# EleutherAI/DALLE-mtf

Hardware: AMD Instinct MI355X
Metric: train tokens/sec (text+image) per node, dalle_example (higher is better)
Workload: dtype bf16

## Files before the change

dalle-mtf_amd/csrc/attention.hip:

```cpp
#include "common.h"
#include <type_traits>
#include <algorithm>
#include <string.h>
#include <vector>

#define HD 128
#define LOG2E_F 1.4426950408889634f
#define KP 136
#define TP 68
#define TP32 36

__device__ __forceinline__ bf16x8 cat4(bf16x4 a, bf16x4 b) { return __builtin_shufflevector(a, b, 0, 1, 2, 3, 4, 5, 6, 7); }
__device__ __forceinline__ bf16x8 pack_bf8(const float* p) {
  u32x4 v = {pack2bf(p[0], p[1]), pack2bf(p[2], p[3]), pack2bf(p[4], p[5]), pack2bf(p[6], p[7])};
  return __builtin_bit_cast(bf16x8, v);
}

template <int ROWS>
__device__ __forceinline__ void load_nat_regs(u32x4* r, const bf16_t* __restrict__ g, int64_t ld, int row0, int nrows, int tid) {
#pragma unroll
  for (int i = 0; i < ROWS / 16; ++i) {
    const int c = tid + 256 * i, row = c >> 4, ch = c & 15;
    int gr = row0 + row;
    gr = gr < nrows ? gr : nrows - 1;
// ... 836 lines not shown
  {
    const int items = ((S + 127) / 128) * B * H;
    const int grid = items < 2 * attn_num_cus() ? items : 2 * attn_num_cus();
    const int perxcd = g_opt_attn_xcd && (B * H) % 8 == 0 && grid % 8 == 0;
    if (g_opt_attn_fwd == 0) attn_fwd_kernel<false><<<dim3(grid), dim3(256), 2 * QK_STAGE, (hipStream_t)stream>>>(qkv, o, lse, B, H, S, perxcd);
#ifdef ATTN_STAMP
    else attn_fwd2_kernel<<<dim3(grid), dim3(256), 2 * QK_STAGE, (hipStream_t)stream>>>(qkv, o, lse, B, H, S, perxcd, g_dbg_buf);
#else
    else attn_fwd2_kernel<<<dim3(grid), dim3(256), 2 * QK_STAGE, (hipStream_t)stream>>>(qkv, o, lse, B, H, S, perxcd);
#endif
  }
  DMI_CHECK_LAUNCH("attention_fwd");
  return DMI_OK;
}

template <int rowstore, bool MASKED, typename... PLAN>
__global__ __launch_bounds__(256, 2) void attn_bwd_dq_kernel(const bf16_t* __restrict__ qkv, const bf16_t* __restrict__ o,
                                                             const bf16_t* __restrict__ d_o, const float* __restrict__ lse,
                                                             float* __restrict__ delta, float* __restrict__ stats,
                                                             bf16_t* __restrict__ dqkv, PLAN __restrict__... plan_, int B, int H, int S, int perxcd) {
  static_assert(sizeof...(PLAN) == (MASKED ? 1 : 0), "the plan pointer is an argument of the masked instance only");
  extern __shared__ __attribute__((aligned(16))) char sm[];
  const int d = H * HD, ld3 = 3 * d;
  int T = (S + 127) / 128, W = 0;
  const int* __restrict__ fptr = nullptr;
  const int* __restrict__ flist = nullptr;
  const int* __restrict__ forder = nullptr;
  const unsigned* __restrict__ rowbits = nullptr;
  if constexpr (MASKED) {
    const int* __restrict__ plan = (plan_, ...);
    T = plan[AMP_NB], W = plan[AMP_W];
    fptr = plan + plan[AMP_FPTR];
    flist = plan + plan[AMP_FLIST];
    forder = plan + plan[AMP_FORDER];
    rowbits = (const unsigned*)(plan + plan[AMP_ROWBITS]);
  }
  const AttnSched sched = attn_sched(T, B * H, perxcd);
  int tile_, bh;
  for (int round = 0; attn_item(sched, round, tile_, bh); ++round) {
// ... 11 lines not shown
  int tid = threadIdx.x;
  asm volatile("" : "+v"(tid));
  const int lane = tid & 63;
  const int wid = __builtin_amdgcn_readfirstlane(tid >> 6);
  const int r = lane & 31, h = lane >> 5, g4 = lane >> 4, l16 = lane & 15;
  const int qrow = q0 + wid * 32 + r;
  const int qrow_c = qrow < S ? qrow : S - 1;
  const unsigned* __restrict__ mrow = nullptr;
  if constexpr (MASKED) mrow = rowbits + (int64_t)qrow_c * W;
  const bf16_t* qb = qkv + (int64_t)b * S * ld3 + hh * HD;
  const bf16_t* dob = d_o + (int64_t)b * S * d + hh * HD;
  const unsigned lds0 = (unsigned)(uintptr_t)(__attribute__((address_space(3))) char*)sm;
  const int nbytes = (int)(((int64_t)(S - 1) * ld3 + HD) * 2);
  const __amdgpu_buffer_rsrc_t rk = __builtin_amdgcn_make_buffer_rsrc((void*)(qb + d), 0, nbytes, 0x00020000);
  const __amdgpu_buffer_rsrc_t rv = __builtin_amdgcn_make_buffer_rsrc((void*)(qb + 2 * d), 0, nbytes, 0x00020000);

  bf16x8 qf[8], dof[8], of_[8];
#pragma unroll
  for (int kk = 0; kk < 8; ++kk) {
    qf[kk] = *(const bf16x8*)(qb + (int64_t)qrow_c * ld3 + 16 * kk + 8 * h);
    dof[kk] = *(const bf16x8*)(dob + (int64_t)qrow_c * d + 16 * kk + 8 * h);
    of_[kk] = *(const bf16x8*)(o + ((int64_t)b * S + qrow_c) * d + hh * HD + 16 * kk + 8 * h);
  }
  const float lse_q = lse[(int64_t)bh * S + qrow_c];
  const float lse2_q = lse_q * LOG2E_F;
  float delta_q = 0.f;
  {
#pragma unroll
    for (int kk = 0; kk < 8; ++kk) {
      float fo[8], fd[8];
      unpack8(__builtin_bit_cast(u32x4, of_[kk]), fo);
      unpack8(__builtin_bit_cast(u32x4, dof[kk]), fd);
#pragma unroll
      for (int j = 0; j < 8; ++j) delta_q += fo[j] * fd[j];
    }
    delta_q += __shfl_xor(delta_q, 32, 64);
    if (h == 0 && qrow < S) {
      const int64_t idx = (int64_t)bh * S + qrow;
      delta[idx] = delta_q;
      stats[2 * idx] = lse2_q;
      stats[2 * idx + 1] = delta_q;
    }
  }

  int vo[4];
#pragma unroll
  for (int i = 0; i < 4; ++i) {
    const int c = tid + 256 * i, row = c >> 4, pc = c & 15;
    vo[i] = (row * ld3 + 8 * (pc ^ swz(row))) * 2;
  }
  auto stage = [&](int st, int key0) {
    char* base = sm + st * QK_STAGE;
#pragma unroll
    for (int i = 0; i < 4; ++i) {
      dma16(rk, base + (wid * 64 + 256 * i) * 16, vo[i] + key0 * ld3 * 2);
      dma16(rv, base + 16384 + (wid * 64 + 256 * i) * 16, vo[i] + key0 * ld3 * 2);
    }
  };
  int ofa[8];
#pragma unroll
  for (int kk = 0; kk < 8; ++kk) ofa[kk] = r * 256 + (((2 * kk + h) ^ swz(r)) << 4);
  const int rr = l16 >> 2;
  unsigned oft0[2];
#pragma unroll
  for (int w2 = 0; w2 < 2; ++w2) {
    const int row = 4 * h + rr + 8 * w2;
    const int chunk = 2 * (g4 & 1) + ((l16 & 3) >> 1);
    oft0[w2] = row * 256 + ((chunk ^ swz(row)) << 4) + 8 * (l16 & 1);
  }

  f32x16 dq[4];
#pragma unroll
// ... 51 lines not shown
      } else {
#pragma unroll
        for (int e = 0; e < 16; ++e) {
          const float pe = __builtin_amdgcn_exp2f(__builtin_fmaf(s[e], LOG2E_F, -lse2_q));
          ds[e] = pe * (dp[e] - delta_q);
        }
      }
      bf16x8 dsb[2];
      dsb[0] = pack_bf8(ds);
      dsb[1] = pack_bf8(ds + 8);
#pragma unroll
      for (int q = 0; q < 4; ++q) {
        const int s2 = q >> 1, dp2 = (q & 1) * 2;
        Tr2& c = tk[q & 1];
        tr2_wait(c);
        if (q < 3) {
          const int s2n = (q + 1) >> 1, dn = ((q + 1) & 1) * 2;
          const unsigned u0 = t0 + s2n * 4096, u1 = t1 + s2n * 4096;
          tr2_issue(tk[(q + 1) & 1], lds0 + (u0 ^ (dn << 6)), lds0 + (u1 ^ (dn << 6)), lds0 + (u0 ^ ((dn + 1) << 6)), lds0 + (u1 ^ ((dn + 1) << 6)));
        }
        dq[dp2] = __builtin_amdgcn_mfma_f32_32x32x16_bf16(cat2(c.a0, c.a1), dsb[s2], dq[dp2], 0, 0, 0);
        dq[dp2 + 1] = __builtin_amdgcn_mfma_f32_32x32x16_bf16(cat2(c.b0, c.b1), dsb[s2], dq[dp2 + 1], 0, 0, 0);
      }
    }
  };

  if constexpr (MASKED) {
    if (nsteps > 0) stage(0, 64 * (list[0] & 0xffff));
    asm volatile("s_waitcnt vmcnt(0)" ::: "memory");
    __syncthreads();
    for (int i = 0; i < nsteps; ++i) {
      const int ent = list[i];
      unsigned b0, b1;
      amp_row_bits(ent, wid, mrow, W, b0, b1);
      if (i + 1 < nsteps) stage((i + 1) & 1, 64 * (list[i + 1] & 0xffff));
      compute(i & 1, ent, b0, b1);
      asm volatile("s_waitcnt vmcnt(0)" ::: "memory");
      __syncthreads();
    }
  } else {
    stage(0, 0);
    asm volatile("s_waitcnt vmcnt(0)" ::: "memory");
    __syncthreads();
    int j = 0;
    for (; j + 2 <= nsteps; j += 2) {
      stage(1, 64 * (j + 1));
      compute(0, j);
      asm volatile("s_waitcnt vmcnt(0)" ::: "memory");
      __syncthreads();
      if (j + 2 < nsteps) stage(0, 64 * (j + 2));
      compute(1, j + 1);
      asm volatile("s_waitcnt vmcnt(0)" ::: "memory");
      __syncthreads();
// ... 38 lines not shown
      "ds_read_b128 %4, %8 offset:128\n\t"
      "ds_read_b128 %5, %8 offset:144\n\t"
      "ds_read_b128 %6, %8 offset:192\n\t"
      "ds_read_b128 %7, %8 offset:208"
      : "=&v"(f.v[0]), "=&v"(f.v[1]), "=&v"(f.v[2]), "=&v"(f.v[3]), "=&v"(f.v[4]), "=&v"(f.v[5]), "=&v"(f.v[6]), "=&v"(f.v[7])
      : "v"(a)
      : "memory");
}
template <int N>
__device__ __forceinline__ void st8_wait(St8& f) {
  asm volatile("s_waitcnt lgkmcnt(%8)"
               : "+v"(f.v[0]), "+v"(f.v[1]), "+v"(f.v[2]), "+v"(f.v[3]), "+v"(f.v[4]), "+v"(f.v[5]), "+v"(f.v[6]), "+v"(f.v[7])
               : "n"(N)
               : "memory");
}
template <int rowstore>
__global__ __launch_bounds__(256, 1) void attn_bwd_dkv_kernel(const bf16_t* __restrict__ qkv, const bf16_t* __restrict__ d_o,
                                                               const float* __restrict__ stats ,
                                                               bf16_t* __restrict__ dqkv, int B, int H, int S, int perxcd) {
  extern __shared__ __attribute__((aligned(16))) char sm[];
  const int d = H * HD, ld3 = 3 * d;
  const AttnSched sched = attn_sched((S + 127) / 128, B * H, perxcd);
  int ktile, bh;
  for (int round = 0; attn_item(sched, round, ktile, bh); ++round) {
  const int b = bh / H, hh = bh % H;
  const int key0 = ktile * 128;
  int tid = threadIdx.x;
  asm volatile("" : "+v"(tid));
  const int lane = tid & 63;
  const int wid = __builtin_amdgcn_readfirstlane(tid >> 6);
  const int r = lane & 31, h = lane >> 5, g4 = lane >> 4, l16 = lane & 15;
  const int krow = key0 + wid * 32 + r;
  const int krow_c = krow < S ? krow : S - 1;
  const bf16_t* qb = qkv + (int64_t)b * S * ld3 + hh * HD;
  const bf16_t* kb = qb + d;
  const bf16_t* vb = qb + 2 * d;
  const bf16_t* dob = d_o + (int64_t)b * S * d + hh * HD;
  const unsigned lds0 = (unsigned)(uintptr_t)(__attribute__((address_space(3))) char*)sm;

  const __amdgpu_buffer_rsrc_t rq = __builtin_amdgcn_make_buffer_rsrc((void*)qb, 0, (int)(((int64_t)(S - 1) * ld3 + HD) * 2), 0x00020000);
  const __amdgpu_buffer_rsrc_t rdo = __builtin_amdgcn_make_buffer_rsrc((void*)dob, 0, (int)(((int64_t)(S - 1) * d + HD) * 2), 0x00020000);
  const __amdgpu_buffer_rsrc_t rv = __builtin_amdgcn_make_buffer_rsrc((void*)vb, 0, (int)(((int64_t)(S - 1) * ld3 + HD) * 2), 0x00020000);
  const __amdgpu_buffer_rsrc_t rst = __builtin_amdgcn_make_buffer_rsrc((void*)(stats + (int64_t)bh * S * 2), 0, S * 8, 0x00020000);

  bf16x8 kf[8];
#pragma unroll
  for (int kk = 0; kk < 8; ++kk) kf[kk] = *(const bf16x8*)(kb + (int64_t)krow_c * ld3 + 16 * kk + 8 * h);

#pragma unroll
  for (int i = 0; i < 8; ++i) {
    const int c = tid + 256 * i, row = c >> 4, pc = c & 15;
    int gr = key0 + row;
    gr = gr < S ? gr : S - 1;
    dma16(rv, sm + (wid * 64 + 256 * i) * 16, (gr * ld3 + 8 * (pc ^ swz(row))) * 2);
  }
  int voq[2], vod[2];
#pragma unroll
  for (int i = 0; i < 2; ++i) {
// ... 146 lines not shown
      if (do_dma) stage_q(st3, q3, 1);
      dk[2] = __builtin_amdgcn_mfma_f32_32x32x16_bf16(cat2(tq.c0, tq.c1), dsb[0], dk[2], 0, 0, 0);
      dk[3] = __builtin_amdgcn_mfma_f32_32x32x16_bf16(cat2(tq.d0, tq.d1), dsb[0], dk[3], 0, 0, 0);
      __builtin_amdgcn_sched_barrier(0);
      tr4_wait8(t2, tq);
      if constexpr (has_next) st8_issue(stt, lds0 + 32768 + so + 16384 + 32 * h);
      dv[0] = __builtin_amdgcn_mfma_f32_32x32x16_bf16(cat2(t2.a0, t2.a1), pb[1], dv[0], 0, 0, 0);
      dv[1] = __builtin_amdgcn_mfma_f32_32x32x16_bf16(cat2(t2.b0, t2.b1), pb[1], dv[1], 0, 0, 0);
      if (do_dma) stage_st(st3, q3);
      dv[2] = __builtin_amdgcn_mfma_f32_32x32x16_bf16(cat2(t2.c0, t2.c1), pb[1], dv[2], 0, 0, 0);
      dv[3] = __builtin_amdgcn_mfma_f32_32x32x16_bf16(cat2(t2.d0, t2.d1), pb[1], dv[3], 0, 0, 0);
      __builtin_amdgcn_sched_barrier(0);
      if constexpr (has_next) tr4_wait8(tdo, t2); else tr4_wait(tdo);
      dk[0] = __builtin_amdgcn_mfma_f32_32x32x16_bf16(cat2(tdo.a0, tdo.a1), dsb[1], dk[0], 0, 0, 0);
      dk[1] = __builtin_amdgcn_mfma_f32_32x32x16_bf16(cat2(tdo.b0, tdo.b1), dsb[1], dk[1], 0, 0, 0);
      dk[2] = __builtin_amdgcn_mfma_f32_32x32x16_bf16(cat2(tdo.c0, tdo.c1), dsb[1], dk[2], 0, 0, 0);
      dk[3] = __builtin_amdgcn_mfma_f32_32x32x16_bf16(cat2(tdo.d0, tdo.d1), dsb[1], dk[3], 0, 0, 0);
      if constexpr (has_next) st8_wait<0>(stt);
    }
  };

  if (nsteps > 0) stage(0, 32 * qi0);
  if (nsteps > 1) stage(1, 32 * (qi0 + 1));
  if (nsteps > 2) stage(2, 32 * (qi0 + 2));
  if (nsteps > 2) DKV_WAIT(5); else DKV_WAIT(0);
  DKV_BARRIER();
  if (nsteps > 0) {
    st8_issue(stt, lds0 + 32768 + 16384 + 32 * h);
    sdp_only(0, sA, dpA);
  }
  int t = 0;
#define DKV_STEP(CS, CD, NS, ND, NEXT, MASK)                                \
  {                                                                         \
    body(t & 3, qi0 + t, t, CS, CD, NS, ND, std::integral_constant<bool, NEXT>{}, std::integral_constant<bool, MASK>{}); \
    if (nsteps - 1 - t >= 3) DKV_WAIT(5); else DKV_WAIT(0);                 \
    DKV_BARRIER();                                                          \
    ++t;                                                                    \
  }
  while (t < 4 && t + 3 <= nsteps) {
    DKV_STEP(sA, dpA, sB, dpB, true, true) DKV_STEP(sB, dpB, sA, dpA, true, true)
  }
  while (t + 3 <= nsteps) {
    DKV_STEP(sA, dpA, sB, dpB, true, false) DKV_STEP(sB, dpB, sA, dpA, true, false)
  }
  if (nsteps - t == 2) {
    DKV_STEP(sA, dpA, sB, dpB, true, true) DKV_STEP(sB, dpB, sA, dpA, false, true)
  } else if (nsteps - t == 1) {
    DKV_STEP(sA, dpA, sB, dpB, false, true)
  }
#undef DKV_STEP
// ... 6 lines not shown
    __syncthreads();
  } else if (krow < S) {
    bf16_t* okp = dqkv + ((int64_t)b * S + krow) * ld3 + d + hh * HD;
    bf16_t* ovp = okp + d;
#pragma unroll
    for (int dt = 0; dt < 4; ++dt)
#pragma unroll
      for (int q4 = 0; q4 < 4; ++q4) {
        const int dd = dt * 32 + 8 * q4 + 4 * h;
        *(u32x2*)(okp + dd) = u32x2{pack2bf(dk[dt][4 * q4], dk[dt][4 * q4 + 1]), pack2bf(dk[dt][4 * q4 + 2], dk[dt][4 * q4 + 3])};
        *(u32x2*)(ovp + dd) = u32x2{pack2bf(dv[dt][4 * q4], dv[dt][4 * q4 + 1]), pack2bf(dv[dt][4 * q4 + 2], dv[dt][4 * q4 + 3])};
      }
  }
  }
}

extern "C" int dmi_attention_bwd(const uint16_t* qkv, const uint16_t* o, const uint16_t* d_o, const float* lse, float* delta,
                                 uint16_t* dqkv, int B, int H, int S, void* stream) {
  DMI_REQUIRE(qkv && o && d_o && lse && delta && dqkv, "attention_bwd: null pointer");
  DMI_REQUIRE(B > 0 && H > 0 && S > 0 && S % 8 == 0, "attention_bwd: S must be a multiple of 8 (S=%d)", S);
  DMI_REQUIRE((int64_t)S * 3 * H * HD * 2 < 0x7fffffff, "attention_bwd: sequence too long for 32-bit buffer offsets");
  hipStream_t st = (hipStream_t)stream;
  float* stats = delta + (int64_t)B * H * S;
  static bool attr_done = false;
  const int shm = 32768 + DKV_NSTAGE * DKV_STAGE;
  if (!attr_done) {
    (void)hipFuncSetAttribute((const void*)attn_bwd_dq_kernel<0, false>, hipFuncAttributeMaxDynamicSharedMemorySize, 2 * QK_STAGE);
    (void)hipFuncSetAttribute((const void*)attn_bwd_dq_kernel<1, false>, hipFuncAttributeMaxDynamicSharedMemorySize, 2 * QK_STAGE);
    (void)hipFuncSetAttribute((const void*)attn_bwd_dkv_kernel<0>, hipFuncAttributeMaxDynamicSharedMemorySize, shm);
    (void)hipFuncSetAttribute((const void*)attn_bwd_dkv_kernel<1>, hipFuncAttributeMaxDynamicSharedMemorySize, shm);
    attr_done = true;
  }
  const int items = ((S + 127) / 128) * B * H;
  {
    const int grid = items < 2 * attn_num_cus() ? items : 2 * attn_num_cus();
    const int perxcd = g_opt_attn_xcd && (B * H) % 8 == 0 && grid % 8 == 0;
    if (g_opt_attn_bwd & 1) attn_bwd_dq_kernel<1, false><<<dim3(grid), dim3(256), 2 * QK_STAGE, st>>>(qkv, o, d_o, lse, delta, stats, dqkv, B, H, S, perxcd);
    else attn_bwd_dq_kernel<0, false><<<dim3(grid), dim3(256), 2 * QK_STAGE, st>>>(qkv, o, d_o, lse, delta, stats, dqkv, B, H, S, perxcd);
  }
  DMI_CHECK_LAUNCH("attention_bwd_dq");
  {
    const int grid = items < attn_num_cus() ? items : attn_num_cus();
    const int perxcd = g_opt_attn_xcd && (B * H) % 8 == 0 && grid % 8 == 0;
    if (g_opt_attn_bwd & 1) attn_bwd_dkv_kernel<1><<<dim3(grid), dim3(256), shm, st>>>(qkv, d_o, stats, dqkv, B, H, S, perxcd);
    else attn_bwd_dkv_kernel<0><<<dim3(grid), dim3(256), shm, st>>>(qkv, d_o, stats, dqkv, B, H, S, perxcd);
  }
  DMI_CHECK_LAUNCH("attention_bwd_dkv");
  return DMI_OK;
}

#define DEC_WAVES 16
template <int STRIDE>
__device__ __forceinline__ float lane_groups_sum(float v) {
  if constexpr (STRIDE < 64) {
    v += __shfl_xor(v, STRIDE, 64);
    return lane_groups_sum<2 * STRIDE>(v);
  }
  return v;
}
template <int HEAD_DIM, bool MASKED, typename... PLAN>
__global__ __launch_bounds__(64 * DEC_WAVES) void attn_decode_kernel(bf16_t* qkv, const bf16_t* __restrict__ fresh, bf16_t* __restrict__ o,
                                                                     PLAN __restrict__... plan_, int H, int S, int pos_arg,
                                                                     const int* __restrict__ pos_dev) {
// ... 1111 lines not shown
```

dalle-mtf_amd/csrc/gemm.hip:

```cpp
#include "common.h"
#include <string.h>
#include <type_traits>

static int g_opt_nt4 = 1;
static int g_opt_nt8 = 1;
int g_opt_reserve_cus = 0;
int g_opt_attn_fwd = 1;
int g_opt_attn_bwd = 1;
int g_opt_attn_mask_force = 0;
int g_opt_attn_xcd = 8;
static int g_opt_tn8 = 0;
static int g_opt_tn8_max_tiles = 16;
static int g_opt_nt8_min_k = 2048;
static int g_opt_skinny = 1;
static int g_opt_tn_wide = 1;
static int g_opt_tn_tail = 1;
static int g_opt_cstream = 1;
static int g_opt_cstream_min_mb = 256;
static int g_opt_cstream_nt_min_mb = 1024;
static int g_opt_res16 = 1;
static int g_opt_ntr = 1;
static int g_opt_nt8p = 1;
static int g_opt_relu_bits = 1;
static int g_opt_nt8p_max_k = 1024;
// ... 3315 lines not shown
```

dalle-mtf_amd/dalle_hip/__init__.py:

```python
from __future__ import annotations

import ctypes
import os
import re
import struct

import numpy as np
from ctypes import c_char_p, c_float, c_int, c_int64, c_uint64, c_void_p

import torch

_HERE = os.path.dirname(os.path.abspath(__file__))
LIB_PATH = os.environ.get("DALLE_HIP_LIB") or os.path.join(_HERE, "libdalle_hip.so")
HEADER_PATH = os.path.join(os.path.dirname(os.path.dirname(_HERE)), "include", "dalle_hip.h")

GEMM_BIAS, GEMM_RELU, GEMM_RESIDUAL, GEMM_RELU_MASK, GEMM_OUT_F32, GEMM_ROWSCALE = 1, 2, 4, 8, 16, 32
GEMM_GELU = 512

_lib = None


class DalleHipError(RuntimeError):
    pass

# ... 52 lines not shown
        "dmi_gemm_nt_splitk_workspace_bytes": (L64, [I, I, I]),
        "dmi_gemm_nt_splitk": (I, [P, I, P, I, P, I, I, I, I, P, P, P]),
        "dmi_gemm_tn_workspace_bytes": (L64, [I, I, I]),
        "dmi_gemm_tn": (I, [P, I, P, I, P, P, P, I, I, I, P, P, P, P]),
        "dmi_gemm_tn_group": (I, [P, I, I, P, P, P]),
        "dmi_gemm_tn_group_plan": (I, [P, P, I, I]),
        "dmi_reduce_slabs_batch": (I, [P, I, P]),
        "dmi_colsum_workspace_bytes": (L64, [L64, I]),
        "dmi_colsum": (I, [P, I, P, L64, I, P, P]),
        "dmi_transpose_bf16": (I, [P, P, I, I, I, P]),
        "dmi_attention_fwd": (I, [P, P, P, I, I, I, P]),
        "dmi_attention_bwd": (I, [P, P, P, P, P, P, I, I, I, P]),
        "dmi_attention_decode": (I, [P, P, P, I, I, I, I, P, P]),
        "dmi_attention_fwd_hd": (I, [P, P, P, I, I, I, I, P]),
        "dmi_attention_bwd_hd": (I, [P, P, P, P, P, P, I, I, I, I, P]),
        "dmi_attention_decode_hd": (I, [P, P, P, I, I, I, I, P, I, P]),
        "dmi_attn_mask_plan": (L64, [P, I, P, L64]),
        "dmi_attention_fwd_masked": (I, [P, P, P, P, P, I, I, I, I, P]),
        "dmi_attention_bwd_masked": (I, [P, P, P, P, P, P, P, P, I, I, I, I, P]),
        "dmi_attention_decode_masked": (I, [P, P, P, P, P, I, I, I, I, P, I, P]),
        "dmi_label_logit": (I, [P, I, P, I, P, P, P, P, L64, I, I, P]),
        "dmi_gemm_nt_softmax_partials": (L64, [I]),
        "dmi_gemm_nt_softmax": (I, [P, I, P, I, P, P, P, I, P, I, I, I, P]),
        "dmi_softmax_finish": (I, [P, I, P, P, P, P, I, P, I, P, P, I, I, P, P, P, P, P, L64, I, I, F, P]),
        "dmi_softmax_finish_w": (I, [P, I, P, P, P, P, I, P, I, P, P, I, I, P, P, P, P, P, L64, I, I, F, P, I, P]),
        "dmi_loss_reduce": (I, [P, L64, P, I, I, F, P, P]),
        "dmi_shift_labels": (I, [P, P, I, I, I, P]),
        "dmi_cross_entropy": (I, [P, I, P, P, P, L64, I, F, P]),
        "dmi_sum_f32": (I, [P, L64, F, P, P]),
        "dmi_assemble_tokens": (I, [P, P, P, I, I, I, I, I, P]),
# ... 428 lines not shown
    _dev(in_base, out_base, table)
    _check(lib().dmi_transpose_bf16_batch(_p(in_base), _p(out_base), _p(table), n, total_tiles, _stream()), "transpose_batch")


def attention_fwd(qkv, o, lse, B, H, S, head_dim=128):
    _dev(qkv, o, lse)
    _check(lib().dmi_attention_fwd_hd(_p(qkv), _p(o), _p(lse), B, H, S, int(head_dim), _stream()), "attention_fwd")


def attention_bwd(qkv, o, d_o, lse, scratch, dqkv, B, H, S, head_dim=128):
    _dev(qkv, o, d_o, lse, scratch, dqkv)
    _check(lib().dmi_attention_bwd_hd(_p(qkv), _p(o), _p(d_o), _p(lse), _p(scratch), _p(dqkv), B, H, S, int(head_dim), _stream()),
           "attention_bwd")


PLAN_MAGIC = 0x504D4144
PLAN_HDR = dict(S=1, NB=2, W=3, CAUSAL=4, FPTR=5, FLIST=6, KPTR=7, KLIST=8, FORDER=9, KORDER=10, ROWBITS=11, COLBITS=12, WORDS=13,
                LIVE_F=14, CAUSAL_F=15, LIVE_K=16, CAUSAL_K=17)


class AttnMaskPlan:

    def __init__(self, mask, device="cuda"):
        m = np.ascontiguousarray(np.asarray(mask.cpu() if hasattr(mask, "cpu") else mask).astype(np.uint8))
        if m.ndim != 2 or m.shape[0] != m.shape[1]:
            raise DalleHipError(f"attn_mask_plan: the mask must be [S, S] (got {m.shape})")
        self.S = int(m.shape[0])
        fn = lib().dmi_attn_mask_plan
        nbytes = fn(m.ctypes.data, self.S, None, 0)
        if nbytes < 0:
# ... 357 lines not shown
```

dalle-mtf_amd/src/dalle_mtf/engine.py:

```python
from __future__ import annotations

import contextlib
import gc
import hashlib
import logging
import math
import os
from collections import OrderedDict, namedtuple
from typing import Dict, Optional, Tuple

import numpy as np
import torch

import dalle_hip as dh
from ..dp import GradReducer
from .activations import check_activation
from .dropout import SITE_POSITION, SITE_TOKEN, resolve_dropout, site_attention, site_key, site_mlp
from .layout import ALIGN, ParamLayout, _round_up, adafactor_factored_dims, adafactor_table, reference_init
from .ff_glu import resolve_ff_glu
from .qk_norm import GAIN_NAMES, resolve_qk_norm
from .ema import ema_decay_at, one_minus_decay, resolve_ema, resolve_weights
from .loss_weights import position_weights, resolve_loss_weights
from .rotary import DEFAULT_BASE, resolve_rotary, rotary_table
from .token_shift import grid_side, resolve_token_shift
# ... 147 lines not shown
            if plan.causal:
                continue
            if self.hd != 128:
                raise dh.DalleHipError(f"custom attention masks need head dim 128 (n_embd/n_heads = {self.hd}); "
                                       "the head-dim-64 kernels implement the causal mask only")
            self.attn_plan[l] = plan

    def _attn_fwd(self, l, qkv, o, lse):
        if self.attn_plan[l] is None:
            dh.attention_fwd(qkv, o, lse, self.B, self.H, self.S, head_dim=self.hd)
        else:
            dh.attention_fwd_masked(qkv, o, lse, self.attn_plan[l], self.B, self.H, self.S, head_dim=self.hd)

    def _attn_bwd(self, l):
        args = (self.qkv[l], self.o[l], self.d_o, self.lse[l], self.delta, self.dqkv)
        if self.attn_plan[l] is None:
            dh.attention_bwd(*args, self.B, self.H, self.S, head_dim=self.hd)
        else:
            dh.attention_bwd_masked(*args, self.attn_plan[l], self.B, self.H, self.S, head_dim=self.hd)

    def _attn_decode(self, l, cache, o, fresh, pos_dev):
        if self.attn_plan[l] is None:
            dh.attention_decode(cache, o, self.B, self.H, self.S, 0, fresh=fresh, pos_dev=pos_dev, head_dim=self.hd)
        else:
            dh.attention_decode_masked(cache, o, self.attn_plan[l], self.B, self.H, self.S, 0, fresh=fresh, pos_dev=pos_dev,
                                       head_dim=self.hd)

    OPTIMIZERS = ("adam", "adafactor")

    def set_optimizer(self, name):
        name = (name or "adam").lower()
# ... 191 lines not shown
        self.tok_sorted = torch.empty(M, dtype=torch.int32, device=self.dev)
        self.tok_perm = torch.empty(M, dtype=torch.int32, device=self.dev)
        self.sort_ws = torch.empty(dh.sort_tokens_workspace_bytes(M), **u8)
        self.embed_ws = torch.empty(dh.embed_bwd_workspace_bytes(B, S, d), **u8)
        self.sort_stream = torch.cuda.Stream(device=self.dev)
        self._sort_done = None
        self.dx = [torch.empty(M, d, **b16) for _ in range(2)]
        self.dxn = torch.empty(M, d, **b16)
        self.dh = torch.empty(M, 4 * d, **b16)
        self.dpre = torch.empty(M, self.F1, **b16) if self.ffn_form == "glu" else None
        self.dqkv = torch.empty(M, 3 * d, **b16)
        self.d_o = torch.empty(M, d, **b16)
        self.drop_y = torch.empty(M, d, **b16) if self.resid_thresh else None
        self.dyd = [torch.empty(M, d, **b16) for _ in range(2)] if self.resid_thresh else None
        self.delta = torch.empty(3, B, H, S, **f32)
        wsz = max(dh.gemm_tn_workspace_bytes(M, d, Vp), *(dh.gemm_tn_workspace_bytes(M, i_, j_) for i_, j_ in self.wgrad_shapes),
                  dh.layernorm_bwd_workspace_bytes(M, d), dh.sumsq_workspace_bytes(self.lay.total),
                  dh.gemm_nt_splitk_workspace_bytes(M // 2 + 256, d, 8),
                  dh.qk_norm_bwd_workspace_bytes(M, self.hd) if self.qk_norm else 0)
        self.ws = torch.empty(int(wsz) + 1024, **u8)
        self.ws_blk = [torch.empty(int(dh.gemm_tn_workspace_bytes(M, i_, j_)) + 256, **u8) for i_, j_ in self.wgrad_shapes]
        self.deferred = dh.DeferredReduces()
        if self.fuse_lnbwd:
            npart = dh.gemm_nt_lnbwd_parts(M) * 2 * d
            self.lnb_part = [torch.empty(npart, **f32) for _ in range(2 * L if self.lnb_batch else 1)]
            self.ln_ws_final = torch.empty(int(dh.layernorm_bwd_workspace_bytes(M, d)) + 256, **u8)

    def _w(self, name):
        return self.view(self.pb, name)

# ... 712 lines not shown
```

include/dalle_hip.h:

```cpp
#ifndef DALLE_HIP_H
#define DALLE_HIP_H
#include <stddef.h>
#include <stdint.h>
#ifdef __cplusplus
extern "C" {
#endif

typedef enum {
  DMI_OK = 0,
  DMI_ERR_INVALID = -1,
  DMI_ERR_LAUNCH = -2,
  DMI_ERR_UNSUPPORTED = -3
} dmi_status;

const char* dmi_last_error_string(void);
int dmi_version(void);
int dmi_get_option(const char* name);
int dmi_set_option(const char* name, int value);
int dmi_set_debug_buffer(void* device_buffer);

int dmi_embed_fwd(const int32_t* tokens, const uint16_t* wte, const uint16_t* wpe, uint16_t* x,
                  int64_t rows , int S, int d, int vocab, const int* pos_dev, void* stream);
int64_t dmi_sort_tokens_workspace_bytes(int64_t n);
int dmi_sort_tokens(const int32_t* tokens, int32_t* sorted_tokens, int32_t* perm, int64_t n, int vocab,
// ... 57 lines not shown
                const uint16_t* bias_weights, int M, int I, int J, void* workspace, dmi_reduce_item* deferred,
                int* n_deferred, void* stream);
int dmi_reduce_slabs_batch(const dmi_reduce_item* items, int n, void* stream);
typedef struct dmi_tn_problem { const uint16_t* X; int ldx; const uint16_t* dY; int ldy; float* dW; float* dbias;
                                const uint16_t* bias_weights; int I; int J; void* workspace; } dmi_tn_problem;
int dmi_gemm_tn_group(const dmi_tn_problem* probs, int n, int M, dmi_reduce_item* deferred, int* n_deferred, void* stream);
int dmi_gemm_tn_group_plan(const int* I, const int* J, int n, int M);

int64_t dmi_colsum_workspace_bytes(int64_t M, int N);
int dmi_colsum(const uint16_t* Y, int ldy, float* out, int64_t M, int N, void* workspace, void* stream);
int dmi_transpose_bf16(const uint16_t* in, uint16_t* out, int batch, int R, int C, void* stream);

int dmi_attention_fwd(const uint16_t* qkv, uint16_t* o, float* lse, int B, int H, int S, void* stream);
int dmi_attention_bwd(const uint16_t* qkv, const uint16_t* o, const uint16_t* d_o, const float* lse, float* scratch,
                      uint16_t* dqkv, int B, int H, int S, void* stream);

int dmi_attention_decode(uint16_t* qkv, const uint16_t* fresh, uint16_t* o, int B, int H, int S, int pos, const int* pos_dev,
                         void* stream);
int dmi_attention_fwd_hd(const uint16_t* qkv, uint16_t* o, float* lse, int B, int H, int S, int head_dim, void* stream);
int dmi_attention_bwd_hd(const uint16_t* qkv, const uint16_t* o, const uint16_t* d_o, const float* lse, float* scratch,
                         uint16_t* dqkv, int B, int H, int S, int head_dim, void* stream);
int dmi_attention_decode_hd(uint16_t* qkv, const uint16_t* fresh, uint16_t* o, int B, int H, int S, int pos, const int* pos_dev,
                            int head_dim, void* stream);

int64_t dmi_attn_mask_plan(const uint8_t* mask, int S, int32_t* plan, int64_t plan_bytes);
int dmi_attention_fwd_masked(const uint16_t* qkv, uint16_t* o, float* lse, const int32_t* plan, const int32_t* plan_host, int B, int H,
                             int S, int head_dim, void* stream);
int dmi_attention_bwd_masked(const uint16_t* qkv, const uint16_t* o, const uint16_t* d_o, const float* lse, float* scratch,
                             uint16_t* dqkv, const int32_t* plan, const int32_t* plan_host, int B, int H, int S, int head_dim,
                             void* stream);
// ... 133 lines not shown
```

Measured before the change: 2.812 million.

## Reuse dS from dK/dV backward pass in dQ kernel via workspace

Restructures the causal attention backward. A separate delta kernel computes the row statistics first. The dK/dV kernel then writes its bf16 dS tiles into a per-(batch, head) global workspace, and a new dQ kernel variant streams K and those stored dS tiles instead of recomputing QK^T, softmax and dP. This removes the duplicated score and dP recomputation in the dQ pass. In exchange it adds global-memory writes and reads of the dS tiles, a large extra workspace allocation, and one more kernel launch. It is enabled by default through the option value change and the engine allocating the workspace.

Result: no change. 2.834 million, median of 6 (+0.8%).

```diff
diff --git a/dalle-mtf_amd/csrc/attention.hip b/dalle-mtf_amd/csrc/attention.hip
--- a/dalle-mtf_amd/csrc/attention.hip
+++ b/dalle-mtf_amd/csrc/attention.hip
@@ -874,15 +874,28 @@
   return DMI_OK;
 }
 
-template <int rowstore, bool MASKED, typename... PLAN>
+#define DS_SUB 2048
+#ifndef DS_STORE_AUX
+#define DS_STORE_AUX 18
+#endif
+#define DS_SLOTS 2
+__host__ __device__ __forceinline__ int ds_sub_base(int kb, int nq32) { return 4 * (kb * nq32 - 2 * kb * (kb - 1)); }
+__device__ __forceinline__ void dma16_s(__amdgpu_buffer_rsrc_t rsrc, char* lds_wave_base, int voff, int soff) {
+  __builtin_amdgcn_raw_ptr_buffer_load_lds(rsrc, (__attribute__((address_space(3))) void*)lds_wave_base, 16, voff, soff, 0, 0);
+}
+template <int form, bool MASKED, typename... PLAN>
 __global__ __launch_bounds__(256, 2) void attn_bwd_dq_kernel(const bf16_t* __restrict__ qkv, const bf16_t* __restrict__ o,
                                                              const bf16_t* __restrict__ d_o, const float* __restrict__ lse,
                                                              float* __restrict__ delta, float* __restrict__ stats,
                                                              bf16_t* __restrict__ dqkv, PLAN __restrict__... plan_, int B, int H, int S, int perxcd) {
-  static_assert(sizeof...(PLAN) == (MASKED ? 1 : 0), "the plan pointer is an argument of the masked instance only");
+  constexpr int rowstore = form & 1;
+  constexpr bool DS = (form & 2) != 0;
+  static_assert(!(DS && MASKED) && (!DS || rowstore), "dQ from dS: the causal whole-row-store instance only");
+  static_assert(sizeof...(PLAN) == (MASKED || DS ? 1 : 0), "the plan / workspace pointer is an argument of the masked / dS instance only");
   extern __shared__ __attribute__((aligned(16))) char sm[];
   const int d = H * HD, ld3 = 3 * d;
   int T = (S + 127) / 128, W = 0;
+  [[maybe_unused]] const int nq32 = (S + 31) / 32;
   const int* __restrict__ fptr = nullptr;
   const int* __restrict__ flist = nullptr;
   const int* __restrict__ forder = nullptr;
@@ -924,8 +937,15 @@
   const int nbytes = (int)(((int64_t)(S - 1) * ld3 + HD) * 2);
   const __amdgpu_buffer_rsrc_t rk = __builtin_amdgcn_make_buffer_rsrc((void*)(qb + d), 0, nbytes, 0x00020000);
   const __amdgpu_buffer_rsrc_t rv = __builtin_amdgcn_make_buffer_rsrc((void*)(qb + 2 * d), 0, nbytes, 0x00020000);
+  [[maybe_unused]] __amdgpu_buffer_rsrc_t rds = rv;
+  if constexpr (DS) {
+    const int ds_bytes = ds_sub_base(T, nq32) * DS_SUB;
+    rds = __builtin_amdgcn_make_buffer_rsrc((void*)((const char*)(plan_, ...) + (int64_t)bh * ds_bytes), 0, ds_bytes, 0x00020000);
+  }
 
   bf16x8 qf[8], dof[8], of_[8];
+  float lse2_q = 0.f, delta_q = 0.f;
+  if constexpr (!DS) {
 #pragma unroll
   for (int kk = 0; kk < 8; ++kk) {
     qf[kk] = *(const bf16x8*)(qb + (int64_t)qrow_c * ld3 + 16 * kk + 8 * h);
@@ -933,8 +953,7 @@
     of_[kk] = *(const bf16x8*)(o + ((int64_t)b * S + qrow_c) * d + hh * HD + 16 * kk + 8 * h);
   }
   const float lse_q = lse[(int64_t)bh * S + qrow_c];
-  const float lse2_q = lse_q * LOG2E_F;
-  float delta_q = 0.f;
+  lse2_q = lse_q * LOG2E_F;
   {
 #pragma unroll
     for (int kk = 0; kk < 8; ++kk) {
@@ -952,6 +971,7 @@
       stats[2 * idx + 1] = delta_q;
     }
   }
+  }
 
   int vo[4];
 #pragma unroll
@@ -966,6 +986,22 @@
       dma16(rk, base + (wid * 64 + 256 * i) * 16, vo[i] + key0 * ld3 * 2);
       dma16(rv, base + 16384 + (wid * 64 + 256 * i) * 16, vo[i] + key0 * ld3 * 2);
     }
+  };
+  [[maybe_unused]] const int qi = 4 * qt + wid;
+  auto ds_live = [&](int j) { return qi < nq32 && 2 * j <= qi; };
+  auto stage_k = [&](int st, int j) {
+#pragma unroll
+    for (int i = 0; i < 4; ++i) dma16(rk, sm + st * 16384 + (wid * 64 + 256 * i) * 16, vo[i] + 64 * j * ld3 * 2);
+  };
+  auto stage_ds = [&](int slot, int j) {
+    const int kb = j >> 1;
+#ifdef ATTN_DBG_DS_CONST
+    const int soff = 0 * kb;
+#else
+    const int soff = (ds_sub_base(kb, nq32) + (qi - 4 * kb) * 4 + 2 * (j & 1)) * DS_SUB;
+#endif
+#pragma unroll
+    for (int i = 0; i < 4; ++i) dma16_s(rds, sm + 32768 + slot * 16384 + wid * 4096 + i * 1024, lane * 16 + i * 1024, soff);
   };
   int ofa[8];
 #pragma unroll
@@ -1047,6 +1083,39 @@
         const int s2 = q >> 1, dp2 = (q & 1) * 2;
         Tr2& c = tk[q & 1];
         tr2_wait(c);
+        if (q < 3) {
+          const int s2n = (q + 1) >> 1, dn = ((q + 1) & 1) * 2;
+          const unsigned u0 = t0 + s2n * 4096, u1 = t1 + s2n * 4096;
+          tr2_issue(tk[(q + 1) & 1], lds0 + (u0 ^ (dn << 6)), lds0 + (u1 ^ (dn << 6)), lds0 + (u0 ^ ((dn + 1) << 6)), lds0 + (u1 ^ ((dn + 1) << 6)));
+        }
+        dq[dp2] = __builtin_amdgcn_mfma_f32_32x32x16_bf16(cat2(c.a0, c.a1), dsb[s2], dq[dp2], 0, 0, 0);
+        dq[dp2 + 1] = __builtin_amdgcn_mfma_f32_32x32x16_bf16(cat2(c.b0, c.b1), dsb[s2], dq[dp2 + 1], 0, 0, 0);
+      }
+    }
+  };
+
+  auto compute_ds = [&](int st, int slot, int j) {
+    if (!ds_live(j)) return;
+    const unsigned ods = lds0 + 32768 + slot * 16384 + wid * 4096 + (g4 & 1) * 1024 + (4 * h + rr) * 32 + (l16 & 1) * 16 + ((l16 & 3) >> 1) * 8;
+#pragma unroll
+    for (int kt2 = 0; kt2 < 2; ++kt2) {
+      Tr2 dsf, tk[2];
+      tr2_issue(dsf, ods + kt2 * DS_SUB, ods + kt2 * DS_SUB + 256, ods + kt2 * DS_SUB + 512, ods + kt2 * DS_SUB + 768);
+      unsigned ob = st * 16384 + kt2 * 8192;
+      asm volatile("" : "+v"(ob));
+      const unsigned t0 = ob + oft0[0], t1 = ob + oft0[1];
+      tr2_issue(tk[0], lds0 + t0, lds0 + t1, lds0 + (t0 ^ 64u), lds0 + (t1 ^ 64u));
+      bf16x8 dsb[2];
+#pragma unroll
+      for (int q = 0; q < 4; ++q) {
+        const int s2 = q >> 1, dp2 = (q & 1) * 2;
+        Tr2& c = tk[q & 1];
+        tr2_wait(c);
+        if (q == 0) {
+          tr2_wait(dsf);
+          dsb[0] = cat2(dsf.a0, dsf.a1);
+          dsb[1] = cat2(dsf.b0, dsf.b1);
+        }
         if (q < 3) {
           const int s2n = (q + 1) >> 1, dn = ((q + 1) & 1) * 2;
           const unsigned u0 = t0 + s2n * 4096, u1 = t1 + s2n * 4096;
@@ -1070,6 +1139,20 @@
       compute(i & 1, ent, b0, b1);
       asm volatile("s_waitcnt vmcnt(0)" ::: "memory");
       __syncthreads();
+    }
+  } else if constexpr (DS) {
+    stage_k(0, 0);
+    if (ds_live(0)) stage_ds(0, 0);
+    asm volatile("s_waitcnt vmcnt(0)" ::: "memory");
+    __syncthreads();
+    for (int j = 0; j < nsteps; ++j) {
+      if (j + 1 < nsteps) {
+        stage_k((j + 1) & 1, j + 1);
+        if (ds_live(j + 1)) stage_ds((j + 1) & 1, j + 1);
+      }
+      compute_ds(j & 1, j & 1, j);
+      asm volatile("s_waitcnt vmcnt(0)" ::: "memory");
+      if (j + 1 < nsteps) __syncthreads();
     }
   } else {
     stage(0, 0);
@@ -1138,10 +1221,10 @@
                : "n"(N)
                : "memory");
 }
-template <int rowstore>
-__global__ __launch_bounds__(256, 1) void attn_bwd_dkv_kernel(const bf16_t* __restrict__ qkv, const bf16_t* __restrict__ d_o,
-                                                               const float* __restrict__ stats ,
-                                                               bf16_t* __restrict__ dqkv, int B, int H, int S, int perxcd) {
+template <int rowstore, bool DS>
+__device__ __forceinline__ void attn_bwd_dkv_body(const bf16_t* __restrict__ qkv, const bf16_t* __restrict__ d_o,
+                                                  const float* __restrict__ stats ,
+                                                  bf16_t* __restrict__ dqkv, char* __restrict__ ws, int B, int H, int S, int perxcd) {
   extern __shared__ __attribute__((aligned(16))) char sm[];
   const int d = H * HD, ld3 = 3 * d;
   const AttnSched sched = attn_sched((S + 127) / 128, B * H, perxcd);
@@ -1166,6 +1249,14 @@
   const __amdgpu_buffer_rsrc_t rdo = __builtin_amdgcn_make_buffer_rsrc((void*)dob, 0, (int)(((int64_t)(S - 1) * d + HD) * 2), 0x00020000);
   const __amdgpu_buffer_rsrc_t rv = __builtin_amdgcn_make_buffer_rsrc((void*)vb, 0, (int)(((int64_t)(S - 1) * ld3 + HD) * 2), 0x00020000);
   const __amdgpu_buffer_rsrc_t rst = __builtin_amdgcn_make_buffer_rsrc((void*)(stats + (int64_t)bh * S * 2), 0, S * 8, 0x00020000);
+  [[maybe_unused]] __amdgpu_buffer_rsrc_t rws = rst;
+  [[maybe_unused]] int ws_item = 0;
+  if constexpr (DS) {
+    const int nq32 = (S + 31) / 32;
+    const int ds_bytes = ds_sub_base((S + 127) / 128, nq32) * DS_SUB;
+    rws = __builtin_amdgcn_make_buffer_rsrc((void*)(ws + (int64_t)bh * ds_bytes), 0, ds_bytes, 0x00020000);
+    ws_item = (ds_sub_base(ktile, nq32) + wid) * DS_SUB;
+  }
 
   bf16x8 kf[8];
 #pragma unroll
@@ -1342,6 +1433,11 @@
       if constexpr (has_next) tr4_wait8(tdo, t2); else tr4_wait(tdo);
       dk[0] = __builtin_amdgcn_mfma_f32_32x32x16_bf16(cat2(tdo.a0, tdo.a1), dsb[1], dk[0], 0, 0, 0);
       dk[1] = __builtin_amdgcn_mfma_f32_32x32x16_bf16(cat2(tdo.b0, tdo.b1), dsb[1], dk[1], 0, 0, 0);
+      if constexpr (DS) {
+        const int so_ds = ws_item + t * (4 * DS_SUB);
+        __builtin_amdgcn_raw_buffer_store_b128(__builtin_bit_cast(u32x4, dsb[0]), rws, r * 32 + h * 16, so_ds, DS_STORE_AUX);
+        __builtin_amdgcn_raw_buffer_store_b128(__builtin_bit_cast(u32x4, dsb[1]), rws, r * 32 + h * 16 + 1024, so_ds, DS_STORE_AUX);
+      }
       dk[2] = __builtin_amdgcn_mfma_f32_32x32x16_bf16(cat2(tdo.c0, tdo.c1), dsb[1], dk[2], 0, 0, 0);
       dk[3] = __builtin_amdgcn_mfma_f32_32x32x16_bf16(cat2(tdo.d0, tdo.d1), dsb[1], dk[3], 0, 0, 0);
       if constexpr (has_next) st8_wait<0>(stt);
@@ -1361,7 +1457,8 @@
 #define DKV_STEP(CS, CD, NS, ND, NEXT, MASK)                                \
   {                                                                         \
     body(t & 3, qi0 + t, t, CS, CD, NS, ND, std::integral_constant<bool, NEXT>{}, std::integral_constant<bool, MASK>{}); \
-    if (nsteps - 1 - t >= 3) DKV_WAIT(5); else DKV_WAIT(0);                 \
+    if constexpr (DS) { if (nsteps - 1 - t >= 3) DKV_WAIT(7); else DKV_WAIT(2); }  \
+    else { if (nsteps - 1 - t >= 3) DKV_WAIT(5); else DKV_WAIT(0); }          \
     DKV_BARRIER();                                                          \
     ++t;                                                                    \
   }
@@ -1398,12 +1495,69 @@
   }
   }
 }
-
-extern "C" int dmi_attention_bwd(const uint16_t* qkv, const uint16_t* o, const uint16_t* d_o, const float* lse, float* delta,
-                                 uint16_t* dqkv, int B, int H, int S, void* stream) {
-  DMI_REQUIRE(qkv && o && d_o && lse && delta && dqkv, "attention_bwd: null pointer");
-  DMI_REQUIRE(B > 0 && H > 0 && S > 0 && S % 8 == 0, "attention_bwd: S must be a multiple of 8 (S=%d)", S);
-  DMI_REQUIRE((int64_t)S * 3 * H * HD * 2 < 0x7fffffff, "attention_bwd: sequence too long for 32-bit buffer offsets");
+template <int rowstore>
+__global__ __launch_bounds__(256, 1) void attn_bwd_dkv_kernel(const bf16_t* __restrict__ qkv, const bf16_t* __restrict__ d_o,
+                                                               const float* __restrict__ stats, bf16_t* __restrict__ dqkv, int B, int H,
+                                                               int S, int perxcd) {
+  attn_bwd_dkv_body<rowstore, false>(qkv, d_o, stats, dqkv, nullptr, B, H, S, perxcd);
+}
+__global__ __launch_bounds__(256, 1) void attn_bwd_dkv_ds_kernel(const bf16_t* __restrict__ qkv, const bf16_t* __restrict__ d_o,
+                                                                  const float* __restrict__ stats, bf16_t* __restrict__ dqkv,
+                                                                  char* __restrict__ ws, int B, int H, int S, int perxcd) {
+  attn_bwd_dkv_body<1, true>(qkv, d_o, stats, dqkv, ws, B, H, S, perxcd);
+}
+
+__global__ __launch_bounds__(256) void attn_bwd_delta_kernel(const bf16_t* __restrict__ o, const bf16_t* __restrict__ d_o,
+                                                             const float* __restrict__ lse, float* __restrict__ delta,
+                                                             float* __restrict__ stats, int B, int H, int S) {
+  __shared__ u32x4 img[4][2][512];
+  const int lane = threadIdx.x & 63, wid = threadIdx.x >> 6;
+  const int64_t nseg = (int64_t)B * S * H, seg0 = ((int64_t)blockIdx.x * 4 + wid) * 32;
+  u32x4 ro[8], rd[8];
+#pragma unroll
+  for (int m = 0; m < 8; ++m) {
+    const int64_t sg = seg0 + 4 * m + (lane >> 4);
+    const bool in = sg < nseg;
+    ro[m] = in ? *(const u32x4*)(o + sg * HD + 8 * (lane & 15)) : u32x4{0, 0, 0, 0};
+    rd[m] = in ? *(const u32x4*)(d_o + sg * HD + 8 * (lane & 15)) : u32x4{0, 0, 0, 0};
+  }
+#pragma unroll
+  for (int m = 0; m < 8; ++m) {
+    const int sl = 4 * m + (lane >> 4), pos = sl * 16 + ((lane & 15) ^ (2 * (sl & 7)));
+    img[wid][0][pos] = ro[m];
+    img[wid][1][pos] = rd[m];
+  }
+  __syncthreads();
+  const int sl = lane >> 1, h = lane & 1;
+  float delta_q = 0.f;
+#pragma unroll
+  for (int kk = 0; kk < 8; ++kk) {
+    float fo[8], fd[8];
+    const int pos = sl * 16 + ((2 * kk + h) ^ (2 * (sl & 7)));
+    unpack8(img[wid][0][pos], fo);
+    unpack8(img[wid][1][pos], fd);
+#pragma unroll
+    for (int j = 0; j < 8; ++j) delta_q += fo[j] * fd[j];
+  }
+  delta_q += __shfl_xor(delta_q, 1, 64);
+  const int64_t sg = seg0 + sl;
+  if (h == 0 && sg < nseg) {
+    const int64_t row = sg / H, b = row / S;
+    const int hh = (int)(sg - row * H);
+    const int64_t idx = (b * H + hh) * S + (row - b * S);
+    delta[idx] = delta_q;
+    stats[2 * idx] = lse[idx] * LOG2E_F;
+    stats[2 * idx + 1] = delta_q;
+  }
+}
+
+static int64_t ds_pair_bytes(int S) { return (int64_t)ds_sub_base((S + 127) / 128, (S + 31) / 32) * DS_SUB; }
+extern "C" int64_t dmi_attention_bwd_workspace_bytes(int B, int H, int S) {
+  if (B <= 0 || H <= 0 || S <= 0 || S > (1 << 20)) return 0;
+  return (int64_t)B * H * ds_pair_bytes(S);
+}
+static int attention_bwd_launch(const uint16_t* qkv, const uint16_t* o, const uint16_t* d_o, const float* lse, float* delta,
+                                uint16_t* dqkv, int B, int H, int S, void* stream, char* ws) {
   hipStream_t st = (hipStream_t)stream;
   float* stats = delta + (int64_t)B * H * S;
   static bool attr_done = false;
@@ -1411,26 +1565,56 @@
   if (!attr_done) {
     (void)hipFuncSetAttribute((const void*)attn_bwd_dq_kernel<0, false>, hipFuncAttributeMaxDynamicSharedMemorySize, 2 * QK_STAGE);
     (void)hipFuncSetAttribute((const void*)attn_bwd_dq_kernel<1, false>, hipFuncAttributeMaxDynamicSharedMemorySize, 2 * QK_STAGE);
+    (void)hipFuncSetAttribute((const void*)attn_bwd_dq_kernel<3, false, const char*>, hipFuncAttributeMaxDynamicSharedMemorySize, 32768 + DS_SLOTS * 16384);
     (void)hipFuncSetAttribute((const void*)attn_bwd_dkv_kernel<0>, hipFuncAttributeMaxDynamicSharedMemorySize, shm);
     (void)hipFuncSetAttribute((const void*)attn_bwd_dkv_kernel<1>, hipFuncAttributeMaxDynamicSharedMemorySize, shm);
+    (void)hipFuncSetAttribute((const void*)attn_bwd_dkv_ds_kernel, hipFuncAttributeMaxDynamicSharedMemorySize, shm);
     attr_done = true;
   }
   const int items = ((S + 127) / 128) * B * H;
-  {
-    const int grid = items < 2 * attn_num_cus() ? items : 2 * attn_num_cus();
-    const int perxcd = g_opt_attn_xcd && (B * H) % 8 == 0 && grid % 8 == 0;
-    if (g_opt_attn_bwd & 1) attn_bwd_dq_kernel<1, false><<<dim3(grid), dim3(256), 2 * QK_STAGE, st>>>(qkv, o, d_o, lse, delta, stats, dqkv, B, H, S, perxcd);
-    else attn_bwd_dq_kernel<0, false><<<dim3(grid), dim3(256), 2 * QK_STAGE, st>>>(qkv, o, d_o, lse, delta, stats, dqkv, B, H, S, perxcd);
-  }
+  const int grid_dq = items < 2 * attn_num_cus() ? items : 2 * attn_num_cus();
+  const int grid_dkv = items < attn_num_cus() ? items : attn_num_cus();
+  const int perxcd_dq = g_opt_attn_xcd && (B * H) % 8 == 0 && grid_dq % 8 == 0;
+  const int perxcd_dkv = g_opt_attn_xcd && (B * H) % 8 == 0 && grid_dkv % 8 == 0;
+  if (ws) {
+    const int64_t nseg = (int64_t)B * S * H;
+    attn_bwd_delta_kernel<<<dim3((unsigned)((nseg + 127) / 128)), dim3(256), 0, st>>>(o, d_o, lse, delta, stats, B, H, S);
+    DMI_CHECK_LAUNCH("attention_bwd_delta");
+    attn_bwd_dkv_ds_kernel<<<dim3(grid_dkv), dim3(256), shm, st>>>(qkv, d_o, stats, dqkv, ws, B, H, S, perxcd_dkv);
+    DMI_CHECK_LAUNCH("attention_bwd_dkv_ds");
+    attn_bwd_dq_kernel<3, false, const char*><<<dim3(grid_dq), dim3(256), 32768 + DS_SLOTS * 16384, st>>>(qkv, o, d_o, lse, delta, stats, dqkv, (const char*)ws, B, H, S, perxcd_dq);
+    DMI_CHECK_LAUNCH("attention_bwd_dq_ds");
+    return DMI_OK;
+  }
+  if (g_opt_attn_bwd & 1) attn_bwd_dq_kernel<1, false><<<dim3(grid_dq), dim3(256), 2 * QK_STAGE, st>>>(qkv, o, d_o, lse, delta, stats, dqkv, B, H, S, perxcd_dq);
+  else attn_bwd_dq_kernel<0, false><<<dim3(grid_dq), dim3(256), 2 * QK_STAGE, st>>>(qkv, o, d_o, lse, delta, stats, dqkv, B, H, S, perxcd_dq);
   DMI_CHECK_LAUNCH("attention_bwd_dq");
-  {
-    const int grid = items < attn_num_cus() ? items : attn_num_cus();
-    const int perxcd = g_opt_attn_xcd && (B * H) % 8 == 0 && grid % 8 == 0;
-    if (g_opt_attn_bwd & 1) attn_bwd_dkv_kernel<1><<<dim3(grid), dim3(256), shm, st>>>(qkv, d_o, stats, dqkv, B, H, S, perxcd);
-    else attn_bwd_dkv_kernel<0><<<dim3(grid), dim3(256), shm, st>>>(qkv, d_o, stats, dqkv, B, H, S, perxcd);
-  }
+  if (g_opt_attn_bwd & 1) attn_bwd_dkv_kernel<1><<<dim3(grid_dkv), dim3(256), shm, st>>>(qkv, d_o, stats, dqkv, B, H, S, perxcd_dkv);
+  else attn_bwd_dkv_kernel<0><<<dim3(grid_dkv), dim3(256), shm, st>>>(qkv, d_o, stats, dqkv, B, H, S, perxcd_dkv);
   DMI_CHECK_LAUNCH("attention_bwd_dkv");
   return DMI_OK;
+}
+extern "C" int dmi_attention_bwd(const uint16_t* qkv, const uint16_t* o, const uint16_t* d_o, const float* lse, float* delta,
+                                 uint16_t* dqkv, int B, int H, int S, void* stream) {
+  DMI_REQUIRE(qkv && o && d_o && lse && delta && dqkv, "attention_bwd: null pointer");
+  DMI_REQUIRE(B > 0 && H > 0 && S > 0 && S % 8 == 0, "attention_bwd: S must be a multiple of 8 (S=%d)", S);
+  DMI_REQUIRE((int64_t)S * 3 * H * HD * 2 < 0x7fffffff, "attention_bwd: sequence too long for 32-bit buffer offsets");
+  return attention_bwd_launch(qkv, o, d_o, lse, delta, dqkv, B, H, S, stream, nullptr);
+}
+extern "C" int dmi_attention_bwd_hd(const uint16_t* qkv, const uint16_t* o, const uint16_t* d_o, const float* lse, float* delta,
+                                    uint16_t* dqkv, int B, int H, int S, int head_dim, void* stream);
+extern "C" int dmi_attention_bwd_ws(const uint16_t* qkv, const uint16_t* o, const uint16_t* d_o, const float* lse, float* delta,
+                                    uint16_t* dqkv, int B, int H, int S, int head_dim, void* stream, void* ws, size_t ws_bytes) {
+  if (!(g_opt_attn_bwd & 2)) return dmi_attention_bwd_hd(qkv, o, d_o, lse, delta, dqkv, B, H, S, head_dim, stream);
+  DMI_REQUIRE(head_dim == HD, "attention_bwd_ws: the dS-kept backward takes head dim 128 (head_dim=%d)", head_dim);
+  DMI_REQUIRE(qkv && o && d_o && lse && delta && dqkv, "attention_bwd_ws: null pointer");
+  DMI_REQUIRE(B > 0 && H > 0 && S > 0 && S % 8 == 0, "attention_bwd_ws: S must be a multiple of 8 (S=%d)", S);
+  DMI_REQUIRE((int64_t)S * 3 * H * HD * 2 < 0x7fffffff, "attention_bwd_ws: sequence too long for 32-bit buffer offsets");
+  DMI_REQUIRE(S <= (1 << 20) && ds_pair_bytes(S) < 0x7fffffff, "attention_bwd_ws: a (batch, head) pair's dS tiles pass 2 GiB (S=%d)", S);
+  DMI_REQUIRE(ws != nullptr, "attention_bwd_ws: null workspace");
+  DMI_REQUIRE((int64_t)ws_bytes >= dmi_attention_bwd_workspace_bytes(B, H, S), "attention_bwd_ws: workspace too small (%lld bytes, need %lld)",
+              (long long)ws_bytes, (long long)dmi_attention_bwd_workspace_bytes(B, H, S));
+  return attention_bwd_launch(qkv, o, d_o, lse, delta, dqkv, B, H, S, stream, (char*)ws);
 }
 
 #define DEC_WAVES 16
diff --git a/dalle-mtf_amd/csrc/gemm.hip b/dalle-mtf_amd/csrc/gemm.hip
--- a/dalle-mtf_amd/csrc/gemm.hip
+++ b/dalle-mtf_amd/csrc/gemm.hip
@@ -6,7 +6,7 @@
 static int g_opt_nt8 = 1;
 int g_opt_reserve_cus = 0;
 int g_opt_attn_fwd = 1;
-int g_opt_attn_bwd = 1;
+int g_opt_attn_bwd = 3;
 int g_opt_attn_mask_force = 0;
 int g_opt_attn_xcd = 8;
 static int g_opt_tn8 = 0;
diff --git a/dalle-mtf_amd/dalle_hip/__init__.py b/dalle-mtf_amd/dalle_hip/__init__.py
--- a/dalle-mtf_amd/dalle_hip/__init__.py
+++ b/dalle-mtf_amd/dalle_hip/__init__.py
@@ -90,6 +90,8 @@
         "dmi_attention_decode": (I, [P, P, P, I, I, I, I, P, P]),
         "dmi_attention_fwd_hd": (I, [P, P, P, I, I, I, I, P]),
         "dmi_attention_bwd_hd": (I, [P, P, P, P, P, P, I, I, I, I, P]),
+        "dmi_attention_bwd_workspace_bytes": (L64, [I, I, I]),
+        "dmi_attention_bwd_ws": (I, [P, P, P, P, P, P, I, I, I, I, P, P, ctypes.c_size_t]),
         "dmi_attention_decode_hd": (I, [P, P, P, I, I, I, I, P, I, P]),
         "dmi_attn_mask_plan": (L64, [P, I, P, L64]),
         "dmi_attention_fwd_masked": (I, [P, P, P, P, P, I, I, I, I, P]),
@@ -548,6 +550,16 @@
            "attention_bwd")
 
 
+def attention_bwd_workspace_bytes(B, H, S):
+    return int(lib().dmi_attention_bwd_workspace_bytes(B, H, S))
+
+
+def attention_bwd_ws(qkv, o, d_o, lse, scratch, dqkv, ws, B, H, S, head_dim=128):
+    _dev(qkv, o, d_o, lse, scratch, dqkv, ws)
+    _check(lib().dmi_attention_bwd_ws(_p(qkv), _p(o), _p(d_o), _p(lse), _p(scratch), _p(dqkv), B, H, S, int(head_dim), _stream(),
+                                      _p(ws), ws.numel() * ws.element_size()), "attention_bwd_ws")
+
+
 PLAN_MAGIC = 0x504D4144
 PLAN_HDR = dict(S=1, NB=2, W=3, CAUSAL=4, FPTR=5, FLIST=6, KPTR=7, KLIST=8, FORDER=9, KORDER=10, ROWBITS=11, COLBITS=12, WORDS=13,
                 LIVE_F=14, CAUSAL_F=15, LIVE_K=16, CAUSAL_K=17)
diff --git a/dalle-mtf_amd/src/dalle_mtf/engine.py b/dalle-mtf_amd/src/dalle_mtf/engine.py
--- a/dalle-mtf_amd/src/dalle_mtf/engine.py
+++ b/dalle-mtf_amd/src/dalle_mtf/engine.py
@@ -185,7 +185,9 @@
 
     def _attn_bwd(self, l):
         args = (self.qkv[l], self.o[l], self.d_o, self.lse[l], self.delta, self.dqkv)
-        if self.attn_plan[l] is None:
+        if self.attn_plan[l] is None and self.attn_ws is not None:
+            dh.attention_bwd_ws(*args, self.attn_ws, self.B, self.H, self.S, head_dim=self.hd)
+        elif self.attn_plan[l] is None:
             dh.attention_bwd(*args, self.B, self.H, self.S, head_dim=self.hd)
         else:
             dh.attention_bwd_masked(*args, self.attn_plan[l], self.B, self.H, self.S, head_dim=self.hd)
@@ -407,6 +409,8 @@
         self.drop_y = torch.empty(M, d, **b16) if self.resid_thresh else None
         self.dyd = [torch.empty(M, d, **b16) for _ in range(2)] if self.resid_thresh else None
         self.delta = torch.empty(3, B, H, S, **f32)
+        ws_bytes = dh.attention_bwd_workspace_bytes(B, H, S) if self.hd == 128 and not self.dp_reserve_cus else 0
+        self.attn_ws = torch.empty(ws_bytes, dtype=torch.uint8, device=self.dev) if 0 < ws_bytes < (B * H) << 31 else None
         wsz = max(dh.gemm_tn_workspace_bytes(M, d, Vp), *(dh.gemm_tn_workspace_bytes(M, i_, j_) for i_, j_ in self.wgrad_shapes),
                   dh.layernorm_bwd_workspace_bytes(M, d), dh.sumsq_workspace_bytes(self.lay.total),
                   dh.gemm_nt_splitk_workspace_bytes(M // 2 + 256, d, 8),
diff --git a/include/dalle_hip.h b/include/dalle_hip.h
--- a/include/dalle_hip.h
+++ b/include/dalle_hip.h
@@ -95,6 +95,9 @@
 int dmi_attention_fwd(const uint16_t* qkv, uint16_t* o, float* lse, int B, int H, int S, void* stream);
 int dmi_attention_bwd(const uint16_t* qkv, const uint16_t* o, const uint16_t* d_o, const float* lse, float* scratch,
                       uint16_t* dqkv, int B, int H, int S, void* stream);
+int64_t dmi_attention_bwd_workspace_bytes(int B, int H, int S);
+int dmi_attention_bwd_ws(const uint16_t* qkv, const uint16_t* o, const uint16_t* d_o, const float* lse, float* scratch,
+                         uint16_t* dqkv, int B, int H, int S, int head_dim, void* stream, void* ws, size_t ws_bytes);
 
 int dmi_attention_decode(uint16_t* qkv, const uint16_t* fresh, uint16_t* o, int B, int H, int S, int pos, const int* pos_dev,
                          void* stream);
```
